# awkrail/svpc

Measured on AMD Instinct MI355X. Metric: train steps/sec (vivt, batch=16, clip_seq=12), higher is better.
Workload: dtype bf16x3; 1 GPU; MODEL_TYPE=vivt train step: N=16 videos/GPU x S=12 clips x Lv=100 frames x F=3072, Lt=22, D=768, H=12, L=6 (enc+step-enc+dec), V=951, A=384, E=10; dropout .1/.1/.4; fwd+bwd+allreduce+clip+BertAdam; mode=bf16x3, global_batch=16, parallelism=dp1, launch=hipGraph replay, gpus_requested=1

## Files before the change

### svpc_amd/csrc/gemm_l32.hip

```cpp
#include "gemm_common.h"
#include <stdlib.h>

typedef __bf16 bf16x8 __attribute__((ext_vector_type(8)));
typedef const void __attribute__((address_space(1))) * l32_gptr;
typedef void __attribute__((address_space(3))) * l32_lptr;

constexpr int L32_BK = 32;
__device__ __attribute__((aligned(16))) const float l32_zeros[4] = {0.f, 0.f, 0.f, 0.f};

template <int N> __device__ __forceinline__ void l32_wait_vmcnt() { asm volatile("s_waitcnt vmcnt(%0)" ::"n"(N) : "memory"); }

template <int R, bool KC>
__device__ __forceinline__ const float* l32_src(const float* P, int ld, int m0, int rows, int k0, int j, int lane) {
    if (KC) {
        const int row = 8 * j + (lane >> 3), pos = lane & 7;
        const int c = pos ^ ((row >> 1) & 7);
        const int gr = min(m0 + row, rows - 1);
        return P + (size_t)gr * ld + k0 + 4 * c;
    } else {
        constexpr int CPR = R / 4;
        const int krow = j * (64 / CPR) + lane / CPR, c = lane % CPR;
        const int gm = min(m0 + 4 * c, rows - 4);
        return P + (size_t)(k0 + krow) * ld + gm;
    }
}

template <int R, bool KC>
__device__ __forceinline__ bf16x8 l32_fragment(const char* __restrict__ img, int row0, int ks, int lane) {
    float f[8];
    if (KC) {
        const int row = row0 + (lane & 31), sw = (row >> 1) & 7;
        const int c0 = 4 * ks + 2 * (lane >> 5);
        const float4 lo = *reinterpret_cast<const float4*>(img + row * 128 + ((c0 ^ sw) << 4));
        const float4 hi = *reinterpret_cast<const float4*>(img + row * 128 + (((c0 + 1) ^ sw) << 4));
// ... 144 lines not shown
#undef L32_KOFS

    const u64 seed = (epi.p_drop > 0.f && splitk == 1) ? epi.seed[0] : 0ull;
    const float inv_keep = epi.p_drop > 0.f ? 1.0f / (1.0f - epi.p_drop) : 1.0f;
    const int l31 = lane & 31, lhi = lane >> 5;
#pragma unroll
    for (int i = 0; i < TM; ++i)
#pragma unroll
        for (int j = 0; j < TN; ++j) {
            const int col = n0 + wc * (BN / 2) + j * 32 + l31;
            if (splitk == 1) {
                float vs[16]; int rs[16], cs[16]; bool oks[16];
#pragma unroll
                for (int e = 0; e < 16; ++e) {
                    const int row = m0 + wr * (BM / 2) + i * 32 + (e & 3) + 8 * (e >> 2) + 4 * lhi;
                    vs[e] = acc[i][j][e]; oks[e] = row < M && col < N; rs[e] = min(row, M - 1); cs[e] = min(col, N - 1);
                }
                epilogue_store_n<16>(vs, rs, cs, oks, C, ldc, epi, seed, inv_keep);
                continue;
            }
            if (col >= N) continue;
#pragma unroll
            for (int e = 0; e < 16; ++e) {
                const int row = m0 + wr * (BM / 2) + i * 32 + (e & 3) + 8 * (e >> 2) + 4 * lhi;
                if (row >= M) continue;
                slabs[((size_t)ks_id * M + row) * N + col] = acc[i][j][e];
            }
        }
}

template <bool A_KC, bool B_KC, int NS = 2, bool X3 = false, bool PRE = false>
__device__ __forceinline__ void l32w_tile(char* l32_smem, const float* __restrict__ A, int lda, const float* __restrict__ B, int ldb,
                                          float* __restrict__ C, int ldc, int M, int N, int K, const Epi& epi, int tm, int tn,
                                          float* __restrict__ asum) {
    constexpr int T = 64, OP = T * L32_BK * 4, STAGE = 2 * OP, PIECES = OP / 1024;
    const int m0 = tm * T, n0 = tn * T;
    float cpre[PRE ? T * T / 256 : 1];
    if constexpr (PRE) {
#pragma unroll
        for (int u = 0; u < T * T / 256; ++u) {
            const int idx = threadIdx.x + 256 * u;
            const int row = m0 + (idx >> 6), col = n0 + (idx & 63);
            cpre[u] = (row < M && col < N) ? C[(size_t)row * ldc + col] : 0.f;
        }
    }
    const bool want_asum = !A_KC && asum != nullptr && tn == 0;
    float bsum = 0.f;
    const int lane = threadIdx.x & 63, wave = threadIdx.x >> 6;
    constexpr bool TAIL = !A_KC && !B_KC;
    const int nk_all = TAIL ? (K + L32_BK - 1) / L32_BK : K / L32_BK;
    const int nk = (nk_all - wave + 3) / 4;
    const int krow0 = wave * L32_BK + lane / (T / 4);
    char* const ring = l32_smem + wave * (NS * STAGE);

    const float* ga[PIECES];
    const float* gb[PIECES];
#pragma unroll
    for (int i = 0; i < PIECES; ++i) {
        ga[i] = l32_src<T, A_KC>(A, lda, m0, M, wave * L32_BK, i, lane);
        gb[i] = l32_src<T, B_KC>(B, ldb, n0, N, wave * L32_BK, i, lane);
    }
    const size_t stepA = 4 * (A_KC ? (size_t)L32_BK : (size_t)L32_BK * lda);
    const size_t stepB = 4 * (B_KC ? (size_t)L32_BK : (size_t)L32_BK * ldb);

    floatx16 acc[2][2];
#pragma unroll
    for (int i = 0; i < 2; ++i)
#pragma unroll
        for (int j = 0; j < 2; ++j)
#pragma unroll
            for (int e = 0; e < 16; ++e) acc[i][j][e] = 0.f;

#define L32W_ISSUE(t)                                                                                                       \
    do {                                                                                                                    \
        char* st = ring + ((t) % NS) * STAGE;                                                                               \
        _Pragma("unroll") for (int i = 0; i < PIECES; ++i) {                                                                \
// ... 41 lines not shown
#pragma unroll
                for (int j = 0; j < 2; ++j) bf[j] = l32_fragment<T, B_KC>(sb, j * 32, ks, lane);
#pragma unroll
                for (int i = 0; i < 2; ++i) {
                    const bf16x8 af = l32_fragment<T, A_KC>(sa, i * 32, ks, lane);
#pragma unroll
                    for (int j = 0; j < 2; ++j) acc[i][j] = __builtin_amdgcn_mfma_f32_32x32x16_bf16(af, bf[j], acc[i][j], 0, 0, 0);
                }
            }
        }
        __builtin_amdgcn_wave_barrier();
    }
#undef L32W_ISSUE

    __syncthreads();
    float* part = reinterpret_cast<float*>(l32_smem) + wave * (T * T);
    float* bpart = reinterpret_cast<float*>(l32_smem) + 4 * T * T;
    if (want_asum) bpart[wave * T + lane] = bsum;
    const int l31 = lane & 31, lhi = lane >> 5;
#pragma unroll
    for (int i = 0; i < 2; ++i)
#pragma unroll
        for (int j = 0; j < 2; ++j)
#pragma unroll
            for (int e = 0; e < 16; ++e) {
                const int r = i * 32 + (e & 3) + 8 * (e >> 2) + 4 * lhi;
                part[r * T + j * 32 + l31] = acc[i][j][e];
            }
    __syncthreads();
    const float* p0 = reinterpret_cast<const float*>(l32_smem);
    const u64 seed = epi.p_drop > 0.f ? epi.seed[0] : 0ull;
    const float inv_keep = epi.p_drop > 0.f ? 1.0f / (1.0f - epi.p_drop) : 1.0f;
    constexpr int NE = T * T / 256;
    float vs[NE]; int rs[NE], cs[NE]; bool oks[NE];
#pragma unroll
    for (int u = 0; u < NE; ++u) {
        const int idx = threadIdx.x + 256 * u;
        const int r = idx >> 6, c = idx & 63;
        const float v = ((p0[idx] + p0[T * T + idx]) + p0[2 * T * T + idx]) + p0[3 * T * T + idx];
        const int row = m0 + r, col = n0 + c;
        if constexpr (PRE) { if (row < M && col < N) C[(size_t)row * ldc + col] = v + cpre[u]; }
        else { vs[u] = v; oks[u] = row < M && col < N; rs[u] = min(row, M - 1); cs[u] = min(col, N - 1); }
    }
    if constexpr (!PRE) epilogue_store_n<NE>(vs, rs, cs, oks, C, ldc, epi, seed, inv_keep);
    if (want_asum && threadIdx.x < T && m0 + (int)threadIdx.x < M) {
        const int i = threadIdx.x;
        asum[m0 + i] += ((bpart[i] + bpart[T + i]) + bpart[2 * T + i]) + bpart[3 * T + i];
    }
}

template <bool A_KC, bool B_KC, bool X3 = false>
__global__ __launch_bounds__(256) void gemm_l32w_kernel(const float* __restrict__ A, int lda, const float* __restrict__ B, int ldb,
                                                        float* __restrict__ C, int ldc, int M, int N, int K, Epi epi, int tiles_m,
                                                        int tiles_n) {
    extern __shared__ __attribute__((aligned(1024))) char l32_smem[];
    const int tile = blockIdx.x;
    const int tm = tile / tiles_n, tn = tile - tm * tiles_n;
    l32w_tile<A_KC, B_KC, 2, X3>(l32_smem, A, lda, B, ldb, C, ldc, M, N, K, epi, tm, tn, nullptr);
}

struct GProb { const float* dz; const float* x; float* dw; float* db; int n_out, n_in, rows, ld_dz, ld_x, ld_dw, tile0, tiles_n; };
constexpr int GROUP_MAX = 48;
struct GArgs { int n; GProb p[GROUP_MAX]; };

template <int NS>
__global__ __launch_bounds__(256) void gemm_group_wgrad_kernel(GArgs g) {
    extern __shared__ __attribute__((aligned(1024))) char l32_smem[];
    int pi = 0;
    while (pi + 1 < g.n && (int)blockIdx.x >= g.p[pi + 1].tile0) ++pi;
    const GProb& q = g.p[pi];
    const int tile = blockIdx.x - q.tile0;
    const int tm = tile / q.tiles_n, tn = tile - tm * q.tiles_n;
    Epi epi{nullptr, ACT_NONE, 0.f, 0u, nullptr, 1, nullptr};
    l32w_tile<false, false, NS, false, true>(l32_smem, q.dz, q.ld_dz, q.x, q.ld_x, q.dw, q.ld_dw, q.n_out, q.n_in, q.rows, epi, tm, tn, q.db);
}


template <bool A_KC, bool B_KC, bool X3 = false>
static int l32w_launch_one(dim3 grid, hipStream_t stream, const float* A, int lda, const float* B, int ldb, float* C, int ldc, int M, int N,
                           int K, Epi epi, int tiles_m, int tiles_n) {
    constexpr int LDS = 4 * 2 * 2 * 64 * L32_BK * 4;
    static bool attr_set = false;
    if (!attr_set) {
        hipError_t e = hipFuncSetAttribute(reinterpret_cast<const void*>(&gemm_l32w_kernel<A_KC, B_KC, X3>),
                                           hipFuncAttributeMaxDynamicSharedMemorySize, LDS);
        if (e != hipSuccess) { svpc_set_error("gemm_l32w: cannot raise the dynamic LDS limit"); return (int)e; }
        attr_set = true;
    }
    hipLaunchKernelGGL((gemm_l32w_kernel<A_KC, B_KC, X3>), grid, dim3(256), LDS, stream, A, lda, B, ldb, C, ldc, M, N, K, epi, tiles_m,
                       tiles_n);
    return 0;
}

template <int BM, int BN, bool A_KC, bool B_KC, int NS, bool X3 = false>
static int l32_launch_one(dim3 grid, hipStream_t stream, const float* A, int lda, const float* B, int ldb, float* C, int ldc, int M, int N,
                          int K, Epi epi, int tiles_m, int tiles_n, int splitk, int k_chunk, float* slabs, int remap) {
    constexpr int LDS = NS * (BM + BN) * L32_BK * 4;
    static bool attr_set = false;
    if (!attr_set) {
        hipError_t e = hipFuncSetAttribute(reinterpret_cast<const void*>(&gemm_l32_kernel<BM, BN, A_KC, B_KC, NS, X3>),
                                           hipFuncAttributeMaxDynamicSharedMemorySize, LDS);
        if (e != hipSuccess) { svpc_set_error("gemm_l32: cannot raise the dynamic LDS limit"); return (int)e; }
        attr_set = true;
    }
    hipLaunchKernelGGL((gemm_l32_kernel<BM, BN, A_KC, B_KC, NS, X3>), grid, dim3(256), LDS, stream, A, lda, B, ldb, C, ldc, M, N, K, epi,
                       tiles_m, tiles_n, splitk, k_chunk, slabs, remap);
    return 0;
}
template <int BM, int BN, int NS, bool X3 = false>
// ... 266 lines not shown
    if (skinny && !b_kc) {
        if (kmax >= 1536) hipLaunchKernelGGL((gemm_group_skinny_kernel<8, false, false>), dim3(tiles), dim3(512), 0, stream, g);
        else hipLaunchKernelGGL((gemm_group_skinny_kernel<4, false, false>), dim3(tiles), dim3(256), 0, stream, g);
        return svpc_check_launch("gemm_group_skinny");
    }
    if (skinny) {
        if (x3) {
            if (kmax >= 1536) hipLaunchKernelGGL((gemm_group_skinny_kernel<8, true>), dim3(tiles), dim3(512), 0, stream, g);
            else hipLaunchKernelGGL((gemm_group_skinny_kernel<4, true>), dim3(tiles), dim3(256), 0, stream, g);
        } else if (kmax >= 1536) hipLaunchKernelGGL((gemm_group_skinny_kernel<8, false>), dim3(tiles), dim3(512), 0, stream, g);
        else hipLaunchKernelGGL((gemm_group_skinny_kernel<4, false>), dim3(tiles), dim3(256), 0, stream, g);
        return svpc_check_launch("gemm_group_skinny");
    }
    if (x3) {
        if (a_kc && b_kc) return gemm_group_go<true, true, true>(g, tiles, stream);
        if (a_kc) return gemm_group_go<true, false, true>(g, tiles, stream);
        if (b_kc) return gemm_group_go<false, true, true>(g, tiles, stream);
        return gemm_group_go<false, false, true>(g, tiles, stream);
    }
    if (a_kc && b_kc) return gemm_group_go<true, true>(g, tiles, stream);
    if (a_kc) return gemm_group_go<true, false>(g, tiles, stream);
    if (b_kc) return gemm_group_go<false, true>(g, tiles, stream);
    return gemm_group_go<false, false>(g, tiles, stream);
}
int svpc_gemm_group(const void* problems, int n, int a_kc, int b_kc, int accumulate, hipStream_t stream) {
    return gemm_group_x(problems, n, a_kc, b_kc, accumulate, 0, stream);
}
int svpc_gemm_group_x3(const void* problems, int n, int a_kc, int b_kc, int accumulate, hipStream_t stream) {
    return gemm_group_x(problems, n, a_kc, b_kc, accumulate, 1, stream);
}

int svpc_gemm_group_wgrad(const void* problems, int n, hipStream_t stream) {
    if (n == 0) return 0;
    SVPC_REQUIRE(n > 0 && n <= GROUP_MAX, "gemm_group_wgrad: 1..48 problems per launch");
    const HostWgradProblem* hp = reinterpret_cast<const HostWgradProblem*>(problems);
    GArgs g{};
    g.n = n;
    int tiles = 0;
    for (int i = 0; i < n; ++i) {
        const HostWgradProblem& h = hp[i];
        SVPC_REQUIRE(h.rows > 0 && h.n_out > 0 && h.n_in > 0 && h.n_out % 4 == 0 && h.n_in % 4 == 0 && h.ld_dz % 4 == 0 && h.ld_x % 4 == 0 &&
                         ((((uintptr_t)h.dz) | ((uintptr_t)h.x)) & 15) == 0,
                     "gemm_group_wgrad: n_out % 4, n_in % 4 and 16-byte aligned rows required (any row count)");
        GProb& q = g.p[i];
        q.dz = h.dz; q.x = h.x; q.dw = h.dw; q.db = h.db; q.n_out = h.n_out; q.n_in = h.n_in; q.rows = h.rows; q.ld_dz = h.ld_dz;
        q.ld_x = h.ld_x; q.ld_dw = h.ld_dw; q.tile0 = tiles; q.tiles_n = ceil_div(h.n_in, 64);
        tiles += ceil_div(h.n_out, 64) * q.tiles_n;
    }
    constexpr int LDS2 = 4 * 2 * 2 * 64 * L32_BK * 4, LDS1 = 4 * 64 * 64 * 4 + 1024;
    static bool attr_set = false;
    if (!attr_set) {
        hipError_t e = hipFuncSetAttribute(reinterpret_cast<const void*>(&gemm_group_wgrad_kernel<2>), hipFuncAttributeMaxDynamicSharedMemorySize,
                                           LDS2);
        if (e == hipSuccess)
            e = hipFuncSetAttribute(reinterpret_cast<const void*>(&gemm_group_wgrad_kernel<1>), hipFuncAttributeMaxDynamicSharedMemorySize, LDS1);
        if (e != hipSuccess) { svpc_set_error("gemm_group_wgrad: cannot raise the dynamic LDS limit"); return (int)e; }
        attr_set = true;
    }
    static int ns_env = -1;
    if (ns_env < 0) { const char* e = getenv("SVPC_GROUP_WGRAD_NS"); ns_env = e ? atoi(e) : 1; }
    const bool one_stage = ns_env != 2;
    if (one_stage) hipLaunchKernelGGL(gemm_group_wgrad_kernel<1>, dim3(tiles), dim3(256), LDS1, stream, g);
    else hipLaunchKernelGGL(gemm_group_wgrad_kernel<2>, dim3(tiles), dim3(256), LDS2, stream, g);
    return svpc_check_launch("gemm_group_wgrad");
}

static int gemm_l32_x(const float* A, int lda, int a_kc, const float* B, int ldb, int b_kc, float* C, int ldc, float* Z, const float* R,
                      const float* G, int gact, int M, int N, int K, const float* bias, int act, float p_drop, unsigned site, const u64* seed,
                      int accumulate, float* workspace, size_t workspace_bytes, int x3, hipStream_t stream);
int svpc_gemm_l32_r(const float* A, int lda, int a_kc, const float* B, int ldb, int b_kc, float* C, int ldc, float* Z, const float* R, int M,
                    int N, int K, const float* bias, int act, float p_drop, unsigned site, const u64* seed, int accumulate,
                    float* workspace, size_t workspace_bytes, hipStream_t stream) {
    return gemm_l32_x(A, lda, a_kc, B, ldb, b_kc, C, ldc, Z, R, nullptr, ACT_NONE, M, N, K, bias, act, p_drop, site, seed, accumulate, workspace,
                      workspace_bytes, 0, stream);
}
int svpc_gemm_l32_rg(const float* A, int lda, int a_kc, const float* B, int ldb, int b_kc, float* C, int ldc, const float* R, const float* G,
                     int gact, int M, int N, int K, int accumulate, float* workspace, size_t workspace_bytes, hipStream_t stream) {
    return gemm_l32_x(A, lda, a_kc, B, ldb, b_kc, C, ldc, nullptr, R, G, gact, M, N, K, nullptr, ACT_NONE, 0.f, 0u, nullptr, accumulate,
                      workspace, workspace_bytes, 0, stream);
}
int svpc_gemm_l32_x3(const float* A, int lda, int a_kc, const float* B, int ldb, int b_kc, float* C, int ldc, float* Z, const float* R, int M,
                     int N, int K, const float* bias, int act, float p_drop, unsigned site, const u64* seed, int accumulate,
                     float* workspace, size_t workspace_bytes, hipStream_t stream) {
    return gemm_l32_x(A, lda, a_kc, B, ldb, b_kc, C, ldc, Z, R, nullptr, ACT_NONE, M, N, K, bias, act, p_drop, site, seed, accumulate, workspace,
                      workspace_bytes, 1, stream);
}
int svpc_gemm_l32(const float* A, int lda, int a_kc, const float* B, int ldb, int b_kc, float* C, int ldc, float* Z, int M, int N, int K,
                  const float* bias, int act, float p_drop, unsigned site, const u64* seed, int accumulate, float* workspace,
                  size_t workspace_bytes, hipStream_t stream) {
    return svpc_gemm_l32_r(A, lda, a_kc, B, ldb, b_kc, C, ldc, Z, nullptr, M, N, K, bias, act, p_drop, site, seed, accumulate, workspace,
                           workspace_bytes, stream);
}
}
static int gemm_l32_x(const float* A, int lda, int a_kc, const float* B, int ldb, int b_kc, float* C, int ldc, float* Z, const float* R,
                      const float* G, int gact, int M, int N, int K, const float* bias, int act, float p_drop, unsigned site, const u64* seed,
                      int accumulate, float* workspace, size_t workspace_bytes, int x3, hipStream_t stream) {
// ... 86 lines not shown
```

### svpc_amd/csrc/layernorm.hip

```cpp
#include "common.h"
#include <stdlib.h>

template <int W, typename T>
struct VecIO;
template <>
struct VecIO<4, float> {
    static __device__ __forceinline__ void load(const float* p, float* v) {
        float4 t = *reinterpret_cast<const float4*>(p);
        v[0] = t.x; v[1] = t.y; v[2] = t.z; v[3] = t.w;
    }
    static __device__ __forceinline__ void store(float* p, const float* v) {
        *reinterpret_cast<float4*>(p) = make_float4(v[0], v[1], v[2], v[3]);
    }
};
template <>
struct VecIO<1, float> {
    static __device__ __forceinline__ void load(const float* p, float* v) { v[0] = p[0]; }
    static __device__ __forceinline__ void store(float* p, const float* v) { p[0] = v[0]; }
};
typedef __bf16 bf16x4_t __attribute__((ext_vector_type(4)));
template <>
struct VecIO<4, __bf16> {
    static __device__ __forceinline__ void load(const __bf16* p, float* v) {
        bf16x4_t t = *reinterpret_cast<const bf16x4_t*>(p);
        v[0] = (float)t[0]; v[1] = (float)t[1]; v[2] = (float)t[2]; v[3] = (float)t[3];
    }
    static __device__ __forceinline__ void store(__bf16* p, const float* v) {
        bf16x4_t t;
        t[0] = (__bf16)v[0]; t[1] = (__bf16)v[1]; t[2] = (__bf16)v[2]; t[3] = (__bf16)v[3];
        *reinterpret_cast<bf16x4_t*>(p) = t;
    }
};
template <>
struct VecIO<1, __bf16> {
// ... 607 lines not shown
        for (; g < G; g += 32) s += partial[(size_t)g * ncols + c];
    }
    red[rg][cl] = s;
    __syncthreads();
    float t = 0.f;
    if (rg == 0) {
        t = red[0][cl];
#pragma unroll
        for (int k = 1; k < 32; ++k) t += red[k][cl];
    }
    return t;
}
__global__ __launch_bounds__(1024) void colsum_finalize_kernel(const float* __restrict__ partial, int G, int ncols,
                                                               float* __restrict__ out, int accumulate) {
    __shared__ float red[32][33];
    const int cl = threadIdx.x & 31, rg = threadIdx.x >> 5;
    const int c = blockIdx.x * 32 + cl;
    const float t = finalize_column(partial, G, ncols, c, rg, red);
    if (rg == 0 && c < ncols) out[c] = accumulate ? out[c] + t : t;
}

__global__ __launch_bounds__(1024) void ln_finalize_kernel(const float* __restrict__ partial, int G, int D, float* __restrict__ dgamma,
                                                           float* __restrict__ dbeta, int accumulate) {
    __shared__ float red[32][33];
    const int cl = threadIdx.x & 31, rg = threadIdx.x >> 5;
    const int c = blockIdx.x * 32 + cl, ncols = 2 * D;
    const float t = finalize_column(partial, G, ncols, c, rg, red);
    if (rg == 0 && c < ncols) {
        float* out = c < D ? dgamma + c : dbeta + (c - D);
        *out = accumulate ? *out + t : t;
    }
}

struct FEntry { const float* partial; float* out0; float* out1; int groups, ncols, split, block0; };
constexpr int FIN_MAX = 64;
struct FArgs { int n; FEntry e[FIN_MAX]; };

__global__ __launch_bounds__(1024) void multi_finalize_kernel(FArgs a) {
    __shared__ float red[32][33];
    int ei = 0;
    while (ei + 1 < a.n && (int)blockIdx.x >= a.e[ei + 1].block0) ++ei;
    const FEntry& en = a.e[ei];
    const int cl = threadIdx.x & 31, rg = threadIdx.x >> 5;
    const int c = ((int)blockIdx.x - en.block0) * 32 + cl;
    const float t = finalize_column(en.partial, en.groups, en.ncols, c, rg, red);
    if (rg == 0 && c < en.ncols) {
        float* out = c < en.split ? en.out0 + c : en.out1 + (c - en.split);
        *out += t;
    }
}

template <int KMAX, typename T>
__global__ __launch_bounds__(256) void bucket_colsum_kernel(const T* __restrict__ x, int ldx, const int* __restrict__ idx,
                                                            int R, int C, int K, int rows_per_chunk, float* __restrict__ partial) {
    const int c = blockIdx.x * 256 + threadIdx.x;
    const int chunk = blockIdx.y;
    const int r0 = chunk * rows_per_chunk;
    const int r1 = min(R, r0 + rows_per_chunk);
    float acc[KMAX];
#pragma unroll
    for (int k = 0; k < KMAX; ++k) acc[k] = 0.f;
    if (c < C) {
        for (int r = r0; r < r1; ++r) {
            const float v = (float)x[(size_t)r * ldx + c];
            const int k = idx ? idx[r] : 0;
#pragma unroll
            for (int kk = 0; kk < KMAX; ++kk) acc[kk] += (kk == k) ? v : 0.f;
        }
#pragma unroll
        for (int k = 0; k < KMAX; ++k)
            if (k < K) partial[((size_t)chunk * K + k) * C + c] = acc[k];
    }
}

template <typename T>
__device__ __forceinline__ void colsum_vec_block(float (*red)[512], const T* __restrict__ x, int ldx, int R, int C, int rows_per_chunk,
                                                 float* __restrict__ partial, int colblock, int chunk) {
    constexpr int V = 16 / sizeof(T);
    typedef float vec16 __attribute__((ext_vector_type(4)));
    typedef __bf16 bf16x8v __attribute__((ext_vector_type(8)));
// ... 251 lines not shown
    if (x_dt == 0) hipLaunchKernelGGL(colsum_vec_kernel<float>, vg, dim3(256), 0, stream, (const float*)xv, ldx, R, C, rpc, partial);
    else hipLaunchKernelGGL(colsum_vec_kernel<__bf16>, vg, dim3(256), 0, stream, (const __bf16*)xv, ldx, R, C, rpc, partial);
    return svpc_check_launch("colsum_partial");
}

struct HostColsumEntry { const void* x; float* partial; int dt, ldx, R, C; };
int svpc_multi_colsum(const void* entries, int n, hipStream_t stream) {
    if (n == 0) return 0;
    SVPC_REQUIRE(n > 0 && n <= CSUM_MAX, "multi_colsum: 1..48 entries per launch");
    const HostColsumEntry* he = reinterpret_cast<const HostColsumEntry*>(entries);
    CArgs a{};
    a.n = n;
    int blocks = 0;
    for (int i = 0; i < n; ++i) {
        const int V = he[i].dt ? 8 : 4;
        SVPC_REQUIRE(he[i].R > 0 && he[i].C % V == 0 && he[i].ldx % V == 0 && ((((uintptr_t)he[i].x)) & 15) == 0,
                     "multi_colsum: 16-byte aligned rows required");
        const int chunks = svpc_colsum_chunks(he[i].R);
        a.e[i].x = he[i].x; a.e[i].partial = he[i].partial; a.e[i].dt = he[i].dt; a.e[i].ldx = he[i].ldx; a.e[i].R = he[i].R;
        a.e[i].C = he[i].C; a.e[i].rpc = ceil_div(he[i].R, chunks); a.e[i].colblocks = ceil_div(he[i].C, 64 * V);
        a.e[i].block0 = blocks;
        blocks += a.e[i].colblocks * chunks;
    }
    hipLaunchKernelGGL(multi_colsum_kernel, dim3(blocks), dim3(256), 0, stream, a);
    return svpc_check_launch("multi_colsum");
}

struct HostFinalizeEntry { const float* partial; float* out0; float* out1; int groups, ncols, split; };
int svpc_multi_finalize_max(void) { return FIN_MAX; }
int svpc_multi_finalize(const void* entries, int n, hipStream_t stream) {
    if (n == 0) return 0;
    SVPC_REQUIRE(n > 0 && n <= FIN_MAX, "multi_finalize: 1..64 entries per launch");
    const HostFinalizeEntry* he = reinterpret_cast<const HostFinalizeEntry*>(entries);
    FArgs a{};
    a.n = n;
    int blocks = 0;
    for (int i = 0; i < n; ++i) {
        a.e[i].partial = he[i].partial; a.e[i].out0 = he[i].out0; a.e[i].out1 = he[i].out1; a.e[i].groups = he[i].groups;
        a.e[i].ncols = he[i].ncols; a.e[i].split = he[i].split; a.e[i].block0 = blocks;
        blocks += ceil_div(he[i].ncols, 32);
    }
    hipLaunchKernelGGL(multi_finalize_kernel, dim3(blocks), dim3(1024), 0, stream, a);
    return svpc_check_launch("multi_finalize");
}

int svpc_bucket_colsum_t(const void* xv, int x_dt, int ldx, const int* idx, int R, int C, int K, float* out, int accumulate,
                         float* workspace, hipStream_t stream) {
    SVPC_REQUIRE(K >= 1 && K <= 8, "bucket_colsum: K must be 1..8");
    if (R == 0 || C == 0) return 0;
    const int chunks = svpc_colsum_chunks(R);
    const int rpc = ceil_div(R, chunks);
    dim3 grid(ceil_div(C, 256), chunks);
    const int V = x_dt ? 8 : 4;
    if (K == 1 && idx == nullptr && C % V == 0 && ldx % V == 0 && ((((uintptr_t)xv)) & 15) == 0) {
        const dim3 vg(ceil_div(C, 64 * V), chunks);
        if (x_dt == 0) hipLaunchKernelGGL(colsum_vec_kernel<float>, vg, dim3(256), 0, stream, (const float*)xv, ldx, R, C, rpc, workspace);
        else hipLaunchKernelGGL(colsum_vec_kernel<__bf16>, vg, dim3(256), 0, stream, (const __bf16*)xv, ldx, R, C, rpc, workspace);
    } else if (x_dt == 0) {
        const float* x = (const float*)xv;
        if (K == 1) hipLaunchKernelGGL((bucket_colsum_kernel<1, float>), grid, dim3(256), 0, stream, x, ldx, idx, R, C, K, rpc, workspace);
        else if (K <= 4) hipLaunchKernelGGL((bucket_colsum_kernel<4, float>), grid, dim3(256), 0, stream, x, ldx, idx, R, C, K, rpc, workspace);
        else hipLaunchKernelGGL((bucket_colsum_kernel<8, float>), grid, dim3(256), 0, stream, x, ldx, idx, R, C, K, rpc, workspace);
    } else {
        const __bf16* x = (const __bf16*)xv;
        if (K == 1) hipLaunchKernelGGL((bucket_colsum_kernel<1, __bf16>), grid, dim3(256), 0, stream, x, ldx, idx, R, C, K, rpc, workspace);
        else if (K <= 4) hipLaunchKernelGGL((bucket_colsum_kernel<4, __bf16>), grid, dim3(256), 0, stream, x, ldx, idx, R, C, K, rpc, workspace);
        else hipLaunchKernelGGL((bucket_colsum_kernel<8, __bf16>), grid, dim3(256), 0, stream, x, ldx, idx, R, C, K, rpc, workspace);
    }
    int rc = svpc_check_launch("bucket_colsum");
    if (rc) return rc;
    hipLaunchKernelGGL(colsum_finalize_kernel, dim3(ceil_div(K * C, 32)), dim3(1024), 0, stream, workspace, chunks, K * C,
                       out, accumulate);
    return svpc_check_launch("bucket_colsum finalize");
}
int svpc_bucket_colsum(const float* x, int ldx, const int* idx, int R, int C, int K, float* out, int accumulate,
// ... 6 lines not shown
```

### svpc_amd/csrc/optimizer.hip

```cpp
#include "common.h"

struct TensorMeta { float* p; float* g; float* m; float* v; float* ema; long long n; float wd; int pad; __bf16* shadow; __bf16* shadow_lo; };

constexpr int OPT_CHUNK = 16384;

__global__ __launch_bounds__(256) void opt_sumsq_kernel(const TensorMeta* __restrict__ meta, const int* __restrict__ chunk_tid,
                                                        const long long* __restrict__ chunk_start, float* __restrict__ partial) {
    __shared__ float red[4];
    const int c = blockIdx.x;
    const TensorMeta t = meta[chunk_tid[c]];
    const long long s = chunk_start[c];
    const long long e = s + OPT_CHUNK < t.n ? s + OPT_CHUNK : t.n;
    float acc = 0.f;
    if ((e - s) == OPT_CHUNK && ((((unsigned long long)(t.g + s)) & 15ull) == 0)) {
        const float4* g4 = reinterpret_cast<const float4*>(t.g + s);
        float4 v[OPT_CHUNK / 4 / 256];
#pragma unroll
        for (int k = 0; k < OPT_CHUNK / 4 / 256; ++k) v[k] = g4[threadIdx.x + 256 * k];
#pragma unroll
        for (int k = 0; k < OPT_CHUNK / 4 / 256; ++k) acc += v[k].x * v[k].x + v[k].y * v[k].y + v[k].z * v[k].z + v[k].w * v[k].w;
    } else {
        for (long long i = s + threadIdx.x; i < e; i += 256) { const float g = t.g[i]; acc += g * g; }
    }
    acc = block_sum_256(acc, red);
    if (threadIdx.x == 0) partial[c] = acc;
}
__global__ __launch_bounds__(256) void opt_norms_kernel(const float* __restrict__ partial, const int* __restrict__ tensor_chunk_off,
                                                        int n_tensors, float* __restrict__ norms_sq) {
    __shared__ float red[4];
    float tot = 0.f;
    for (int t = threadIdx.x; t < n_tensors; t += 256) {
        float s = 0.f;
        for (int c = tensor_chunk_off[t]; c < tensor_chunk_off[t + 1]; ++c) s += partial[c];
        norms_sq[t] = s;
        tot += s;
    }
    tot = block_sum_256(tot, red);
    if (threadIdx.x == 0) norms_sq[n_tensors] = tot;
}
__global__ __launch_bounds__(256) void opt_adam_kernel(const TensorMeta* __restrict__ meta, const int* __restrict__ chunk_tid,
                                                       const long long* __restrict__ chunk_start, const float* __restrict__ norms_sq,
                                                       int n_tensors, const float* __restrict__ hyper) {
    const int c = blockIdx.x;
    const int tid = chunk_tid[c];
    const TensorMeta t = meta[tid];
    const float lr = hyper[0], ema_decay = hyper[1], max_g = hyper[2], max_t = hyper[3], b1 = hyper[4], b2 = hyper[5], eps = hyper[6];
    float coef = 1.0f;
    if (max_g > 0.f) coef = fminf(1.0f, max_g / (sqrtf(norms_sq[n_tensors]) + 1e-6f));
    if (max_t > 0.f) {
        const float tn = sqrtf(norms_sq[tid]) * coef;
        coef *= fminf(1.0f, max_t / (tn + 1e-6f));
    }
    const long long s = chunk_start[c];
    const long long e = s + OPT_CHUNK < t.n ? s + OPT_CHUNK : t.n;
    const bool use_ema = t.ema && ema_decay >= 0.f;
    const unsigned long long al = (unsigned long long)(t.g + s) | (unsigned long long)(t.m + s) | (unsigned long long)(t.v + s) |
                                  (unsigned long long)(t.p + s) | (use_ema ? (unsigned long long)(t.ema + s) : 0ull) |
                                  ((t.shadow ? (unsigned long long)(t.shadow + s) : 0ull) << 1) |
                                  ((t.shadow && t.shadow_lo ? (unsigned long long)(t.shadow_lo + s) : 0ull) << 1);
    if ((e - s) == OPT_CHUNK && (al & 15ull) == 0) {
        constexpr int NB = 4, PER = OPT_CHUNK / 4 / 256 / NB;
        float4* __restrict__ g4 = reinterpret_cast<float4*>(t.g + s);
        float4* __restrict__ m4 = reinterpret_cast<float4*>(t.m + s);
        float4* __restrict__ v4 = reinterpret_cast<float4*>(t.v + s);
        float4* __restrict__ p4 = reinterpret_cast<float4*>(t.p + s);
        float4* __restrict__ e4 = reinterpret_cast<float4*>(t.ema + s);
        uint2* __restrict__ sh = reinterpret_cast<uint2*>(t.shadow + s);
        uint2* __restrict__ sl = reinterpret_cast<uint2*>(t.shadow_lo + s);
        for (int b = 0; b < NB; ++b) {
            float4 g[PER], m[PER], v[PER], p[PER], em[PER];
#pragma unroll
// ... 44 lines not shown
        float p = t.p[i];
        float upd = m / (sqrtf(v) + eps);
        if (t.wd > 0.f) upd += t.wd * p;
        p -= lr * upd;
        t.m[i] = m; t.v[i] = v; t.p[i] = p;
        if (t.shadow) {
            const __bf16 ph = (__bf16)p;
            t.shadow[i] = ph;
            if (t.shadow_lo) t.shadow_lo[i] = (__bf16)(p - (float)ph);
        }
        if (t.ema && ema_decay >= 0.f) t.ema[i] = (1.f - ema_decay) * p + ema_decay * t.ema[i];
    }
}
__global__ __launch_bounds__(256) void opt_zero_kernel(const TensorMeta* __restrict__ meta, const int* __restrict__ chunk_tid,
                                                       const long long* __restrict__ chunk_start) {
    const int c = blockIdx.x;
    const TensorMeta t = meta[chunk_tid[c]];
    const long long s = chunk_start[c];
    const long long e = s + OPT_CHUNK < t.n ? s + OPT_CHUNK : t.n;
    for (long long i = s + threadIdx.x; i < e; i += 256) t.g[i] = 0.f;
}

extern "C" {

int svpc_opt_chunk(void) { return OPT_CHUNK; }
int svpc_opt_meta_bytes(void) { return (int)sizeof(TensorMeta); }

int svpc_opt_step(const void* meta, const int* chunk_tid, const long long* chunk_start, const int* tensor_chunk_off, int n_tensors,
                  int n_chunks, float* partial, float* norms_sq, const float* hyper, hipStream_t s) {
    if (n_chunks == 0) return 0;
    hipLaunchKernelGGL(opt_sumsq_kernel, dim3(n_chunks), dim3(256), 0, s, (const TensorMeta*)meta, chunk_tid, chunk_start, partial);
    int rc = svpc_check_launch("opt_sumsq");
    if (rc) return rc;
    hipLaunchKernelGGL(opt_norms_kernel, dim3(1), dim3(256), 0, s, partial, tensor_chunk_off, n_tensors, norms_sq);
    rc = svpc_check_launch("opt_norms");
    if (rc) return rc;
    hipLaunchKernelGGL(opt_adam_kernel, dim3(n_chunks), dim3(256), 0, s, (const TensorMeta*)meta, chunk_tid, chunk_start, norms_sq,
                       n_tensors, hyper);
    return svpc_check_launch("opt_adam");
}
int svpc_opt_zero_grad(const void* meta, const int* chunk_tid, const long long* chunk_start, int n_chunks, hipStream_t s) {
    if (n_chunks == 0) return 0;
    hipLaunchKernelGGL(opt_zero_kernel, dim3(n_chunks), dim3(256), 0, s, (const TensorMeta*)meta, chunk_tid, chunk_start);
    return svpc_check_launch("opt_zero");
}

}
```

Measured before the change: 89.68 steps/s (one step = 16 clip-sequences per GPU; whole-job aggregate).

## Balance grouped wgrad across XCDs, vectorize finalize and epilogue, parallelize optimizer norms

```diff
diff --git a/svpc_amd/csrc/gemm_l32.hip b/svpc_amd/csrc/gemm_l32.hip
--- a/svpc_amd/csrc/gemm_l32.hip
+++ b/svpc_amd/csrc/gemm_l32.hip
@@ -1,5 +1,7 @@
 #include "gemm_common.h"
 #include <stdlib.h>
+#include <string.h>
+#include <algorithm>
 
 typedef __bf16 bf16x8 __attribute__((ext_vector_type(8)));
 typedef const void __attribute__((address_space(1))) * l32_gptr;
@@ -210,16 +212,27 @@
 template <bool A_KC, bool B_KC, int NS = 2, bool X3 = false, bool PRE = false>
 __device__ __forceinline__ void l32w_tile(char* l32_smem, const float* __restrict__ A, int lda, const float* __restrict__ B, int ldb,
                                           float* __restrict__ C, int ldc, int M, int N, int K, const Epi& epi, int tm, int tn,
-                                          float* __restrict__ asum) {
+                                          float* __restrict__ asum, bool c16 = false) {
     constexpr int T = 64, OP = T * L32_BK * 4, STAGE = 2 * OP, PIECES = OP / 1024;
     const int m0 = tm * T, n0 = tn * T;
     float cpre[PRE ? T * T / 256 : 1];
     if constexpr (PRE) {
-#pragma unroll
-        for (int u = 0; u < T * T / 256; ++u) {
-            const int idx = threadIdx.x + 256 * u;
-            const int row = m0 + (idx >> 6), col = n0 + (idx & 63);
-            cpre[u] = (row < M && col < N) ? C[(size_t)row * ldc + col] : 0.f;
+        if (c16) {
+#pragma unroll
+            for (int u = 0; u < T * T / 1024; ++u) {
+                const int qd = threadIdx.x + 256 * u;
+                const int row = m0 + (qd >> 4), col = n0 + 4 * (qd & 15);
+                float4 v = make_float4(0.f, 0.f, 0.f, 0.f);
+                if (row < M && col < N) v = *reinterpret_cast<const float4*>(C + (size_t)row * ldc + col);
+                cpre[4 * u] = v.x; cpre[4 * u + 1] = v.y; cpre[4 * u + 2] = v.z; cpre[4 * u + 3] = v.w;
+            }
+        } else {
+#pragma unroll
+            for (int u = 0; u < T * T / 256; ++u) {
+                const int idx = threadIdx.x + 256 * u;
+                const int row = m0 + (idx >> 6), col = n0 + (idx & 63);
+                cpre[u] = (row < M && col < N) ? C[(size_t)row * ldc + col] : 0.f;
+            }
         }
     }
     const bool want_asum = !A_KC && asum != nullptr && tn == 0;
@@ -327,6 +340,28 @@
     const u64 seed = epi.p_drop > 0.f ? epi.seed[0] : 0ull;
     const float inv_keep = epi.p_drop > 0.f ? 1.0f / (1.0f - epi.p_drop) : 1.0f;
     constexpr int NE = T * T / 256;
+    if constexpr (PRE) {
+        if (c16) {
+            const float4* p4 = reinterpret_cast<const float4*>(l32_smem);
+#pragma unroll
+            for (int u = 0; u < NE / 4; ++u) {
+                const int qd = threadIdx.x + 256 * u;
+                const float4 a = p4[qd], b = p4[T * T / 4 + qd], c = p4[2 * (T * T / 4) + qd], d = p4[3 * (T * T / 4) + qd];
+                const int row = m0 + (qd >> 4), col = n0 + 4 * (qd & 15);
+                float4 o;
+                o.x = (((a.x + b.x) + c.x) + d.x) + cpre[4 * u];
+                o.y = (((a.y + b.y) + c.y) + d.y) + cpre[4 * u + 1];
+                o.z = (((a.z + b.z) + c.z) + d.z) + cpre[4 * u + 2];
+                o.w = (((a.w + b.w) + c.w) + d.w) + cpre[4 * u + 3];
+                if (row < M && col < N) *reinterpret_cast<float4*>(C + (size_t)row * ldc + col) = o;
+            }
+            if (want_asum && threadIdx.x < T && m0 + (int)threadIdx.x < M) {
+                const int i = threadIdx.x;
+                asum[m0 + i] += ((bpart[i] + bpart[T + i]) + bpart[2 * T + i]) + bpart[3 * T + i];
+            }
+            return;
+        }
+    }
     float vs[NE]; int rs[NE], cs[NE]; bool oks[NE];
 #pragma unroll
     for (int u = 0; u < NE; ++u) {
@@ -354,22 +389,25 @@
     l32w_tile<A_KC, B_KC, 2, X3>(l32_smem, A, lda, B, ldb, C, ldc, M, N, K, epi, tm, tn, nullptr);
 }
 
-struct GProb { const float* dz; const float* x; float* dw; float* db; int n_out, n_in, rows, ld_dz, ld_x, ld_dw, tile0, tiles_n; };
+struct GProb { const float* dz; const float* x; float* dw; float* db; int n_out, n_in, rows, ld_dz, ld_x, ld_dw, tile0, tiles_n, c16; };
 constexpr int GROUP_MAX = 48;
-struct GArgs { int n; GProb p[GROUP_MAX]; };
+struct GArgs { int n; int by_xcd; int xcd_tile0[9]; GProb p[GROUP_MAX]; };
 
 template <int NS>
 __global__ __launch_bounds__(256) void gemm_group_wgrad_kernel(GArgs g) {
     extern __shared__ __attribute__((aligned(1024))) char l32_smem[];
+    const int xcd = blockIdx.x & 7;
+    const int gtile = g.by_xcd ? g.xcd_tile0[xcd] + (int)(blockIdx.x >> 3) : (int)blockIdx.x;
+    if (g.by_xcd && gtile >= g.xcd_tile0[xcd + 1]) return;
     int pi = 0;
-    while (pi + 1 < g.n && (int)blockIdx.x >= g.p[pi + 1].tile0) ++pi;
+    while (pi + 1 < g.n && gtile >= g.p[pi + 1].tile0) ++pi;
     const GProb& q = g.p[pi];
-    const int tile = blockIdx.x - q.tile0;
+    const int tile = gtile - q.tile0;
     const int tm = tile / q.tiles_n, tn = tile - tm * q.tiles_n;
     Epi epi{nullptr, ACT_NONE, 0.f, 0u, nullptr, 1, nullptr};
-    l32w_tile<false, false, NS, false, true>(l32_smem, q.dz, q.ld_dz, q.x, q.ld_x, q.dw, q.ld_dw, q.n_out, q.n_in, q.rows, epi, tm, tn, q.db);
-}
-
+    l32w_tile<false, false, NS, false, true>(l32_smem, q.dz, q.ld_dz, q.x, q.ld_x, q.dw, q.ld_dw, q.n_out, q.n_in, q.rows, epi, tm, tn, q.db,
+                                             q.c16 != 0);
+}
 
 template <bool A_KC, bool B_KC, bool X3 = false>
 static int l32w_launch_one(dim3 grid, hipStream_t stream, const float* A, int lda, const float* B, int ldb, float* C, int ldc, int M, int N,
@@ -702,19 +740,33 @@
 
 int svpc_gemm_group_wgrad(const void* problems, int n, hipStream_t stream) {
     if (n == 0) return 0;
-    SVPC_REQUIRE(n > 0 && n <= GROUP_MAX, "gemm_group_wgrad: 1..48 problems per launch");
+    SVPC_REQUIRE(n > 0, "gemm_group_wgrad: a negative problem count");
     const HostWgradProblem* hp = reinterpret_cast<const HostWgradProblem*>(problems);
-    GArgs g{};
-    g.n = n;
-    int tiles = 0;
+    if (n > GROUP_MAX) {
+        for (int i = 0; i < n; i += GROUP_MAX) {
+            const int rc = svpc_gemm_group_wgrad(hp + i, std::min(GROUP_MAX, n - i), stream);
+            if (rc) return rc;
+        }
+        return 0;
+    }
     for (int i = 0; i < n; ++i) {
         const HostWgradProblem& h = hp[i];
         SVPC_REQUIRE(h.rows > 0 && h.n_out > 0 && h.n_in > 0 && h.n_out % 4 == 0 && h.n_in % 4 == 0 && h.ld_dz % 4 == 0 && h.ld_x % 4 == 0 &&
                          ((((uintptr_t)h.dz) | ((uintptr_t)h.x)) & 15) == 0,
                      "gemm_group_wgrad: n_out % 4, n_in % 4 and 16-byte aligned rows required (any row count)");
+    }
+    const char* env = getenv("SVPC_GROUP_WGRAD");
+    GArgs g{};
+    g.n = n;
+    const bool fast = !(env && strcmp(env, "old") == 0);
+    g.by_xcd = fast;
+    int tiles = 0;
+    for (int i = 0; i < n; ++i) {
+        const HostWgradProblem& h = hp[i];
         GProb& q = g.p[i];
         q.dz = h.dz; q.x = h.x; q.dw = h.dw; q.db = h.db; q.n_out = h.n_out; q.n_in = h.n_in; q.rows = h.rows; q.ld_dz = h.ld_dz;
         q.ld_x = h.ld_x; q.ld_dw = h.ld_dw; q.tile0 = tiles; q.tiles_n = ceil_div(h.n_in, 64);
+        q.c16 = fast && h.ld_dw % 4 == 0 && (((uintptr_t)h.dw) & 15) == 0;
         tiles += ceil_div(h.n_out, 64) * q.tiles_n;
     }
     constexpr int LDS2 = 4 * 2 * 2 * 64 * L32_BK * 4, LDS1 = 4 * 64 * 64 * 4 + 1024;
@@ -730,8 +782,26 @@
     static int ns_env = -1;
     if (ns_env < 0) { const char* e = getenv("SVPC_GROUP_WGRAD_NS"); ns_env = e ? atoi(e) : 1; }
     const bool one_stage = ns_env != 2;
-    if (one_stage) hipLaunchKernelGGL(gemm_group_wgrad_kernel<1>, dim3(tiles), dim3(256), LDS1, stream, g);
-    else hipLaunchKernelGGL(gemm_group_wgrad_kernel<2>, dim3(tiles), dim3(256), LDS2, stream, g);
+    int grid = tiles;
+    if (g.by_xcd) {
+        long long work = 0, acc = 0;
+        for (int i = 0; i < n; ++i) work += (long long)(g.p[i].tiles_n * ceil_div(hp[i].n_out, 64)) * (ceil_div(hp[i].rows, L32_BK) + 2);
+        int x = 1, gt = 0, longest = 0;
+        g.xcd_tile0[0] = 0;
+        for (int i = 0; i < n; ++i) {
+            const long long w = ceil_div(hp[i].rows, L32_BK) + 2;
+            const int t = g.p[i].tiles_n * ceil_div(hp[i].n_out, 64);
+            for (int k = 0; k < t; ++k, ++gt) {
+                while (x < 8 && acc * 8 >= work * x) g.xcd_tile0[x++] = gt;
+                acc += w;
+            }
+        }
+        while (x <= 8) g.xcd_tile0[x++] = tiles;
+        for (int k = 0; k < 8; ++k) longest = std::max(longest, g.xcd_tile0[k + 1] - g.xcd_tile0[k]);
+        grid = 8 * longest;
+    }
+    if (one_stage) hipLaunchKernelGGL(gemm_group_wgrad_kernel<1>, dim3(grid), dim3(256), LDS1, stream, g);
+    else hipLaunchKernelGGL(gemm_group_wgrad_kernel<2>, dim3(grid), dim3(256), LDS2, stream, g);
     return svpc_check_launch("gemm_group_wgrad");
 }
 
diff --git a/svpc_amd/csrc/layernorm.hip b/svpc_amd/csrc/layernorm.hip
--- a/svpc_amd/csrc/layernorm.hip
+++ b/svpc_amd/csrc/layernorm.hip
@@ -1,5 +1,6 @@
 #include "common.h"
 #include <stdlib.h>
+#include <string.h>
 
 template <int W, typename T>
 struct VecIO;
@@ -673,7 +674,7 @@
     }
 }
 
-struct FEntry { const float* partial; float* out0; float* out1; int groups, ncols, split, block0; };
+struct FEntry { const float* partial; float* out0; float* out1; int groups, ncols, split, block0, vec; };
 constexpr int FIN_MAX = 64;
 struct FArgs { int n; FEntry e[FIN_MAX]; };
 
@@ -687,6 +688,63 @@
     const float t = finalize_column(en.partial, en.groups, en.ncols, c, rg, red);
     if (rg == 0 && c < en.ncols) {
         float* out = c < en.split ? en.out0 + c : en.out1 + (c - en.split);
+        *out += t;
+    }
+}
+
+constexpr int FIN_VEC_COLS = 128;
+__global__ __launch_bounds__(1024) void multi_finalize_v4_kernel(FArgs a) {
+    __shared__ float red_mem[32 * (FIN_VEC_COLS + 1)];
+    int ei = 0;
+    while (ei + 1 < a.n && (int)blockIdx.x >= a.e[ei + 1].block0) ++ei;
+    const FEntry& en = a.e[ei];
+    const int G = en.groups, ncols = en.ncols;
+    if (!en.vec) {
+        float (*red)[33] = reinterpret_cast<float (*)[33]>(red_mem);
+        const int cl = threadIdx.x & 31, rg = threadIdx.x >> 5;
+        const int c = ((int)blockIdx.x - en.block0) * 32 + cl;
+        const float t = finalize_column(en.partial, G, ncols, c, rg, red);
+        if (rg == 0 && c < ncols) {
+            float* out = c < en.split ? en.out0 + c : en.out1 + (c - en.split);
+            *out += t;
+        }
+        return;
+    }
+    float (*red)[FIN_VEC_COLS + 1] = reinterpret_cast<float (*)[FIN_VEC_COLS + 1]>(red_mem);
+    const int q = threadIdx.x & 31, rg = threadIdx.x >> 5;
+    const int c0 = ((int)blockIdx.x - en.block0) * FIN_VEC_COLS;
+    const int c = c0 + 4 * q;
+    float4 s = make_float4(0.f, 0.f, 0.f, 0.f);
+    if (c < ncols) {
+        const float* __restrict__ p = en.partial + c;
+        int g = rg;
+        for (; g + 224 < G; g += 256) {
+            float4 v[8];
+#pragma unroll
+            for (int k = 0; k < 8; ++k) v[k] = *reinterpret_cast<const float4*>(p + (size_t)(g + 32 * k) * ncols);
+#pragma unroll
+            for (int k = 0; k < 8; ++k) { s.x += v[k].x; s.y += v[k].y; s.z += v[k].z; s.w += v[k].w; }
+        }
+        for (; g + 96 < G; g += 128) {
+            float4 v[4];
+#pragma unroll
+            for (int k = 0; k < 4; ++k) v[k] = *reinterpret_cast<const float4*>(p + (size_t)(g + 32 * k) * ncols);
+#pragma unroll
+            for (int k = 0; k < 4; ++k) { s.x += v[k].x; s.y += v[k].y; s.z += v[k].z; s.w += v[k].w; }
+        }
+        for (; g < G; g += 32) {
+            const float4 v = *reinterpret_cast<const float4*>(p + (size_t)g * ncols);
+            s.x += v.x; s.y += v.y; s.z += v.z; s.w += v.w;
+        }
+    }
+    red[rg][4 * q] = s.x; red[rg][4 * q + 1] = s.y; red[rg][4 * q + 2] = s.z; red[rg][4 * q + 3] = s.w;
+    __syncthreads();
+    const int cc = c0 + (int)threadIdx.x;
+    if (threadIdx.x < FIN_VEC_COLS && cc < ncols) {
+        float t = red[0][threadIdx.x];
+#pragma unroll
+        for (int k = 1; k < 32; ++k) t += red[k][threadIdx.x];
+        float* out = cc < en.split ? en.out0 + cc : en.out1 + (cc - en.split);
         *out += t;
     }
 }
@@ -1004,15 +1062,19 @@
     if (n == 0) return 0;
     SVPC_REQUIRE(n > 0 && n <= FIN_MAX, "multi_finalize: 1..64 entries per launch");
     const HostFinalizeEntry* he = reinterpret_cast<const HostFinalizeEntry*>(entries);
+    const char* env = getenv("SVPC_MULTI_FINALIZE");
+    const bool v4 = !(env && strcmp(env, "old") == 0);
     FArgs a{};
     a.n = n;
     int blocks = 0;
     for (int i = 0; i < n; ++i) {
         a.e[i].partial = he[i].partial; a.e[i].out0 = he[i].out0; a.e[i].out1 = he[i].out1; a.e[i].groups = he[i].groups;
         a.e[i].ncols = he[i].ncols; a.e[i].split = he[i].split; a.e[i].block0 = blocks;
-        blocks += ceil_div(he[i].ncols, 32);
-    }
-    hipLaunchKernelGGL(multi_finalize_kernel, dim3(blocks), dim3(1024), 0, stream, a);
+        a.e[i].vec = v4 && he[i].ncols % 4 == 0 && (((uintptr_t)he[i].partial) & 15) == 0;
+        blocks += ceil_div(he[i].ncols, a.e[i].vec ? FIN_VEC_COLS : 32);
+    }
+    if (v4) hipLaunchKernelGGL(multi_finalize_v4_kernel, dim3(blocks), dim3(1024), 0, stream, a);
+    else hipLaunchKernelGGL(multi_finalize_kernel, dim3(blocks), dim3(1024), 0, stream, a);
     return svpc_check_launch("multi_finalize");
 }
 
diff --git a/svpc_amd/csrc/optimizer.hip b/svpc_amd/csrc/optimizer.hip
--- a/svpc_amd/csrc/optimizer.hip
+++ b/svpc_amd/csrc/optimizer.hip
@@ -1,4 +1,6 @@
 #include "common.h"
+#include <stdlib.h>
+#include <string.h>
 
 struct TensorMeta { float* p; float* g; float* m; float* v; float* ema; long long n; float wd; int pad; __bf16* shadow; __bf16* shadow_lo; };
 
@@ -37,6 +39,56 @@
     }
     tot = block_sum_256(tot, red);
     if (threadIdx.x == 0) norms_sq[n_tensors] = tot;
+}
+__device__ int opt_norms_ticket = 0;
+__global__ __launch_bounds__(256) void opt_norms_wave_kernel(const float* __restrict__ partial, const int* __restrict__ tensor_chunk_off,
+                                                             int n_tensors, float* __restrict__ norms_sq) {
+    __shared__ float red[4];
+    __shared__ int s_last;
+    const int lane = threadIdx.x & 63, wave = __builtin_amdgcn_readfirstlane(threadIdx.x >> 6);
+    const int t = blockIdx.x * 4 + wave;
+    if (t < n_tensors) {
+        const int c0 = tensor_chunk_off[t], c1 = tensor_chunk_off[t + 1];
+        float s = 0.f;
+        for (int b = c0; b < c1; b += 512) {
+            float v[8];
+#pragma unroll
+            for (int k = 0; k < 8; ++k) { const int c = b + 64 * k + lane; v[k] = c < c1 ? partial[c] : 0.f; }
+#pragma unroll
+            for (int k = 0; k < 8; ++k) {
+                const int left = c1 - (b + 64 * k);
+                if (left >= 64) {
+#pragma unroll
+                    for (int i = 0; i < 64; ++i) s += __builtin_bit_cast(float, __builtin_amdgcn_readlane(__builtin_bit_cast(int, v[k]), i));
+                } else {
+                    for (int i = 0; i < left; ++i) s += __builtin_bit_cast(float, __builtin_amdgcn_readlane(__builtin_bit_cast(int, v[k]), i));
+                }
+            }
+        }
+        if (lane == 0) norms_sq[t] = s;
+    }
+    asm volatile("s_waitcnt vmcnt(0)" ::: "memory");
+    __syncthreads();
+    if (threadIdx.x == 0) {
+        __builtin_amdgcn_fence(__ATOMIC_RELEASE, "agent");
+        asm volatile("s_waitcnt vmcnt(0)" ::: "memory");
+        const int ticket = __hip_atomic_fetch_add(&opt_norms_ticket, 1, __ATOMIC_RELAXED, __HIP_MEMORY_SCOPE_AGENT);
+        s_last = ticket == (int)gridDim.x - 1;
+    }
+    __syncthreads();
+    if (!s_last) return;
+    if (threadIdx.x == 0) {
+        __builtin_amdgcn_fence(__ATOMIC_ACQUIRE, "agent");
+        asm volatile("s_waitcnt vmcnt(0)" ::: "memory");
+    }
+    __syncthreads();
+    float tot = 0.f;
+    for (int i = threadIdx.x; i < n_tensors; i += 256) tot += __hip_atomic_load(norms_sq + i, __ATOMIC_RELAXED, __HIP_MEMORY_SCOPE_AGENT);
+    tot = block_sum_256(tot, red);
+    if (threadIdx.x == 0) {
+        norms_sq[n_tensors] = tot;
+        __hip_atomic_store(&opt_norms_ticket, 0, __ATOMIC_RELAXED, __HIP_MEMORY_SCOPE_AGENT);
+    }
 }
 __global__ __launch_bounds__(256) void opt_adam_kernel(const TensorMeta* __restrict__ meta, const int* __restrict__ chunk_tid,
                                                        const long long* __restrict__ chunk_start, const float* __restrict__ norms_sq,
@@ -147,7 +199,11 @@
     hipLaunchKernelGGL(opt_sumsq_kernel, dim3(n_chunks), dim3(256), 0, s, (const TensorMeta*)meta, chunk_tid, chunk_start, partial);
     int rc = svpc_check_launch("opt_sumsq");
     if (rc) return rc;
-    hipLaunchKernelGGL(opt_norms_kernel, dim3(1), dim3(256), 0, s, partial, tensor_chunk_off, n_tensors, norms_sq);
+    const char* env = getenv("SVPC_OPT_NORMS");
+    if (env && strcmp(env, "old") == 0)
+        hipLaunchKernelGGL(opt_norms_kernel, dim3(1), dim3(256), 0, s, partial, tensor_chunk_off, n_tensors, norms_sq);
+    else
+        hipLaunchKernelGGL(opt_norms_wave_kernel, dim3((n_tensors + 3) / 4), dim3(256), 0, s, partial, tensor_chunk_off, n_tensors, norms_sq);
     rc = svpc_check_launch("opt_norms");
     if (rc) return rc;
     hipLaunchKernelGGL(opt_adam_kernel, dim3(n_chunks), dim3(256), 0, s, (const TensorMeta*)meta, chunk_tid, chunk_start, norms_sq,
```

New measurement: 89.67 steps/s (one step = 16 clip-sequences per GPU; whole-job aggregate), median of 2. No clear change (-0.0%).
